# askerlee/segtran

Measured on NVIDIA H100. Metric: voxels/sec fwd+bwd Segtran3d BraTS 112^3 bs=4 hot path, higher is better.
Workload: dtype tf32

## Files before the change

segtran_b200/csrc/sx_gemm.cu:

```cuda
#include <algorithm>
#include <string>

#include "sx_common.cuh"
#include "sx_tc.cuh"

namespace {
using namespace sxtc;

constexpr int NUM_THREADS = 384;
constexpr int STAGES = 4;
constexpr int XPOSE_WARPS = 3;
constexpr int BN_WIDE = 256;
constexpr int CT_LD = 68;
constexpr int CT_WG_FLOATS = 32 * CT_LD;

template <int ES, bool A_MN, bool B_MN, int BN_T>
struct Plan {
  static_assert(BN_T == BN || (BN_T == BN_WIDE && ES == 4 && !A_MN && !B_MN),
                "sx_gemm: the 256-column tile is instantiated for K-major tf32 operands only");
  static constexpr int B_BYTES = BN_T * BKB;
  static constexpr int STAGE_BYTES = A_STAGE_BYTES + B_BYTES;
  static constexpr bool XA = ES == 4 && A_MN, XB = ES == 4 && B_MN;
  static constexpr bool XPOSE = XA || XB;
  static constexpr int RAW_BYTES = (XA ? A_STAGE_BYTES : 0) + (XB ? B_STAGE_BYTES : 0);
// ... 269 lines not shown
    for (int h = 0; h < 2; ++h) {
      const int grow = row0 + 8 * h + tr;
      const float* ar = base + zoff + (long long)(grow < p.M ? grow : 0) * p.ldc;
#pragma unroll
      for (int j = 0; j < 4; ++j) {
        const int col = col0 + 8 * j + tc;
        const int i0 = 4 * j + 2 * h;
        if (grow < p.M && col + 1 < p.N && p.c_vec_ok) {
          const float2 v = *reinterpret_cast<const float2*>(ar + col);
          g[i0] = v.x; g[i0 + 1] = v.y;
        } else {
          g[i0] = (grow < p.M && col < p.N) ? ar[col] : 0.f;
          g[i0 + 1] = (grow < p.M && col + 1 < p.N) ? ar[col + 1] : 0.f;
        }
      }
    }
  };

  const float drop_scale = p.drop_p > 0.f ? 1.f / (1.f - p.drop_p) : 1.f;
  const uint32_t drop_p16v = sx::drop_p16(p.drop_p);
  const unsigned long long drop_seed = p.drop_p > 0.f ? p.drop_seed + (p.drop_seed_dev ? *p.drop_seed_dev : 0ull) : 0ull;
  const uint32_t drop_mul_t = sx::drop_mul((tc >> 1) & 1), drop_key_t = sx::drop_key(drop_seed, (tc >> 1) & 1);

  float acc[BN_T / 2];
  for (int t = blockIdx.x; t < p.total_tiles; t += gridDim.x) {
    int z0, z1, mb, nb, ks;
    decode(t, z0, z1, mb, nb, ks);
    const int nq = p.z1_loop * split_kbs(ks);

    int prev = -1;
    for (int q = 0; q < nq; ++q) {
      sx::mbar_wait(&full_bar[stage], phase);
      const uint8_t* sa = smem + stage * STAGE_BYTES;
      const uint8_t* sb = sa + A_STAGE_BYTES;
      sx::acc_fence(acc);
      sx::wgmma_fence();
#pragma unroll
      for (int kk = 0; kk < KSTEPS; ++kk) {
        const uint64_t da = desc_a(sa, kk, A_MN && !kTF32), db = desc_b(sb, kk, B_MN && !kTF32);
        const uint32_t accum = (q > 0 || kk > 0) ? 1u : 0u;
        if constexpr (WIDE) sx::wgmma_tf32_n256(acc, da, db, accum);
        else if constexpr (kTF32) sx::wgmma_tf32(acc, da, db, accum);
        else sx::wgmma_bf16<A_MN ? 1 : 0, B_MN ? 1 : 0>(acc, da, db, accum);
      }
      sx::wgmma_commit();
      sx::acc_fence(acc);
      sx::wgmma_wait<1>();
      if (prev >= 0 && wtid == 0) sx::mbar_arrive(&empty_bar[prev]);
      prev = stage;
      if (++stage == STAGES) { stage = 0; phase ^= 1; }
    }
    sx::wgmma_wait<0>();
    sx::acc_fence(acc);
    if (prev >= 0 && wtid == 0) sx::mbar_arrive(&empty_bar[prev]);

    const long long zoff = (long long)z1 * p.c_sz1 + (long long)z0 * p.c_sz0;
    const float* bias = p.bias ? p.bias + (long long)z1 * p.bias_sz1 + (long long)z0 * p.bias_sz0 : nullptr;
    const bool add_bias = (bias != nullptr) && (ks == 0);
    const int row0 = mb * BM + cw * 64 + wq * 16;
    float tmax = -3.0e38f;
    float bias_m[2] = {0.f, 0.f};
    if (add_bias && p.bias_mode == SX_BIAS_M) {
#pragma unroll
      for (int h = 0; h < 2; ++h) {
        const int r = row0 + 8 * h + tr;
        bias_m[h] = r < p.M ? bias[r] : 0.f;
      }
    }
    constexpr int EPI_UNROLL = WIDE ? 1 : BN_T / 32;
#pragma unroll EPI_UNROLL
    for (int c = 0; c < BN_T / 32; ++c) {
      const int col0 = nb * BN_T + c * 32;
      if (col0 >= p.N) break;
      float f[16];
#pragma unroll
      for (int i = 0; i < 16; ++i) f[i] = acc[(WIDE ? 0 : 16 * c) + i] * p.alpha + bias_m[(i >> 1) & 1];
      if (p.addend) {
        float g[16];
        load_frag(p.addend, g, zoff, row0, col0);
#pragma unroll
        for (int i = 0; i < 16; ++i) f[i] += g[i];
      }
      if (add_bias && p.bias_mode == SX_BIAS_N) {
#pragma unroll
        for (int j = 0; j < 4; ++j) {
          const int col = col0 + 8 * j + tc;
          const float b0 = col < p.N ? bias[col] : 0.f, b1 = col + 1 < p.N ? bias[col + 1] : 0.f;
#pragma unroll
          for (int h = 0; h < 2; ++h) {
            f[4 * j + 2 * h] += b0;
            f[4 * j + 2 * h + 1] += b1;
          }
        }
      }
      auto apply_dropout = [&]() {
        if (p.drop_p > 0.f) {
          if (((p.ldc | zoff) & 3) == 0) {
#pragma unroll
            for (int h = 0; h < 2; ++h) {
              const unsigned long long g0 =
                  (unsigned long long)((zoff + (long long)(row0 + 8 * h + tr) * p.ldc + col0 + tc) >> 2);
#pragma unroll
              for (int j = 0; j < 4; ++j) {
                const uint32_t bits = sx::drop_word_k(drop_mul_t, drop_key_t, g0 + 2 * j);
                const int i0 = 4 * j + 2 * h;
                f[i0] = (bits & 0xFFFFu) >= drop_p16v ? f[i0] * drop_scale : 0.f;
                f[i0 + 1] = (bits >> 16) >= drop_p16v ? f[i0 + 1] * drop_scale : 0.f;
              }
            }
          } else {
#pragma unroll
            for (int h = 0; h < 2; ++h) {
              const long long rbase = zoff + (long long)(row0 + 8 * h + tr) * p.ldc;
#pragma unroll
              for (int j = 0; j < 4; ++j) {
                const unsigned long long e0 = (unsigned long long)(rbase + col0 + 8 * j + tc);
                const int i0 = 4 * j + 2 * h;
                f[i0] = sx::drop_keep1(drop_seed, e0, drop_p16v) ? f[i0] * drop_scale : 0.f;
                f[i0 + 1] = sx::drop_keep1(drop_seed, e0 + 1, drop_p16v) ? f[i0 + 1] * drop_scale : 0.f;
              }
            }
          }
        }
      };
      if (p.act == SX_ACT_GELU_BWD) {
        apply_dropout();
        float g[16];
        load_frag(reinterpret_cast<const float*>(p.preact), g, zoff, row0, col0);
#pragma unroll
        for (int i = 0; i < 16; ++i) f[i] *= sx::gelu_erf_grad(g[i]);
      } else {
        if (p.preact) store_frag(p.preact, f, zoff, row0, col0, false);
        if (p.act == SX_ACT_GELU) {
#pragma unroll
          for (int i = 0; i < 16; ++i) f[i] = sx::gelu_erf(f[i]);
        }
        apply_dropout();
      }
      if (p.round_tf32 && !p.c_bf16) {
#pragma unroll
        for (int i = 0; i < 16; ++i) f[i] = sx::round_tf32(f[i]);
      }
      if (p.amax) {
#pragma unroll
        for (int h = 0; h < 2; ++h)
          if (row0 + 8 * h + tr < p.M) {
#pragma unroll
            for (int j = 0; j < 4; ++j)
#pragma unroll
              for (int e = 0; e < 2; ++e)
                if (col0 + 8 * j + tc + e < p.N) tmax = fmaxf(tmax, f[4 * j + 2 * h + e]);
          }
      }
      if (!WIDE && p.split_k > 1) {
        float* pt = p.part + ((((long long)z1 * p.Z0 + z0) * p.tiles_m + mb) * p.tiles_n + nb) * p.split_k * (BM * BN) +
                    (long long)ks * (BM * BN);
#pragma unroll
        for (int h = 0; h < 2; ++h)
#pragma unroll
          for (int j = 0; j < 4; ++j)
            *reinterpret_cast<float2*>(pt + (row0 - mb * BM + 8 * h + tr) * BN + (col0 - nb * BN) + 8 * j + tc) =
                make_float2(f[4 * j + 2 * h], f[4 * j + 2 * h + 1]);
      } else {
        store_frag(p.C, f, zoff, row0, col0, p.accumulate != 0);
      }
      if constexpr (PL::CT) {
        if (p.ct) {
          float* cs = ct_stage + cw * CT_WG_FLOATS;
          named_bar_sync(1 + cw);
#pragma unroll
          for (int j = 0; j < 4; ++j)
#pragma unroll
            for (int h = 0; h < 2; ++h)
#pragma unroll
              for (int e = 0; e < 2; ++e) cs[(8 * j + tc + e) * CT_LD + wq * 16 + 8 * h + tr] = f[4 * j + 2 * h + e];
          named_bar_sync(1 + cw);
          const int m0 = mb * BM + cw * 64;
          const long long ctz = (long long)z1 * p.ct_sz1 + (long long)z0 * p.ct_sz0;
#pragma unroll
          for (int i = 0; i < 4; ++i) {
            const int v = wtid + 128 * i, n = v >> 4, r = (v & 15) * 4;
            const int gn = col0 + n, gm = m0 + r;
            if (gn < p.N && gm < p.M) {
              const float4 x = *reinterpret_cast<const float4*>(cs + n * CT_LD + r);
              float* o = p.ct + ctz + (long long)gn * p.ldct + gm;
              if (gm + 3 < p.M) {
                if (p.stream_out) __stcs(reinterpret_cast<float4*>(o), x);
                else *reinterpret_cast<float4*>(o) = x;
              } else {
                o[0] = x.x;
                if (gm + 1 < p.M) o[1] = x.y;
                if (gm + 2 < p.M) o[2] = x.z;
              }
            }
          }
        }
      }
      if constexpr (WIDE) {
#pragma unroll
        for (int i = 0; i < BN_T / 2 - 16; ++i) acc[i] = acc[i + 16];
      }
    }
    if (p.amax) {
      tmax = sx::warp_max(tmax);
      if (lane == 0 && tmax > -3.0e38f) sx::atomic_max_float(p.amax, tmax);
    }
  }
}

__global__ void split_reduce_kernel(const GemmParams p) {
  const long long total = (long long)p.total_tiles / p.split_k * (BM * BN);
  for (long long i = (long long)blockIdx.x * blockDim.x + threadIdx.x; i < total; i += (long long)gridDim.x * blockDim.x) {
    const int e = (int)(i % (BM * BN));
    long long t = i / (BM * BN);
    const int nb = (int)(t % p.tiles_n); t /= p.tiles_n;
    const int mb = (int)(t % p.tiles_m); t /= p.tiles_m;
    const int z0 = (int)(t % p.Z0), z1 = (int)(t / p.Z0);
    const int row = mb * BM + e / BN, col = nb * BN + e % BN;
    if (row >= p.M || col >= p.N) continue;
    const float* pt = p.part + (i / (BM * BN)) * p.split_k * (BM * BN) + e;
    float s = 0.f;
    for (int ks = 0; ks < p.split_k; ++ks) s += pt[(long long)ks * (BM * BN)];
    reinterpret_cast<float*>(p.C)[(long long)z1 * p.c_sz1 + (long long)z0 * p.c_sz0 + (long long)row * p.ldc + col] += s;
  }
}

long long g_max_ctas = -1;
int g_wide_tiles = -1;

template <int ES, bool A_MN, bool B_MN, int BN_T = BN>
int launch(const CUtensorMap& ta, const CUtensorMap& tb, const GemmParams& p, int grid, cudaStream_t st) {
  auto kern = sx_gemm_kernel<ES, A_MN, B_MN, BN_T>;
  constexpr int bytes = Plan<ES, A_MN, B_MN, BN_T>::SMEM;
  SX_CHECK_CUDA(set_max_smem_once(kern, bytes));
  kern<<<grid, NUM_THREADS, bytes, st>>>(ta, tb, p);
  SX_CHECK_CUDA(cudaGetLastError());
  if (p.split_k > 1) {
    const long long n = (long long)p.total_tiles / p.split_k * (BM * BN);
    split_reduce_kernel<<<(int)std::min<long long>(sx_ceil_div(n, 256), 65535), 256, 0, st>>>(p);
    SX_CHECK_CUDA(cudaGetLastError());
  }
  return 0;
}

}

extern "C" int sx_gemm_debug_set(const char* key, int64_t value) {
  std::string k(key);
  if (k == "max_ctas") g_max_ctas = value;
  else if (k == "wide_tiles") g_wide_tiles = value < 0 ? -1 : (value ? 1 : 0);
  else {
    sx_set_error("sx_gemm_debug_set: unknown key %s", key);
    return -1;
  }
  return 0;
}

static int gemm_run(const sx_gemm_args* a, const sx_gemm_tout* t, void* stream) {
  SX_REQUIRE(a != nullptr, "sx_gemm: null args");
  SX_REQUIRE(a->M > 0 && a->N > 0 && a->K > 0 && a->Z0 > 0 && a->Z1 > 0, "sx_gemm: bad shape M=%d N=%d K=%d Z=%dx%d",
             a->M, a->N, a->K, a->Z0, a->Z1);
  SX_REQUIRE(a->op_dtype == SX_OP_TF32 || a->op_dtype == SX_OP_BF16, "sx_gemm: bad op_dtype %d", a->op_dtype);
  SX_REQUIRE(a->C != nullptr && a->A.ptr != nullptr && a->B.ptr != nullptr, "sx_gemm: null pointer");
  const int es = a->op_dtype == SX_OP_TF32 ? 4 : 2;
  const int bk = BKB / es;
  const int sms = sm_count_cached();
  SX_REQUIRE(sms > 0, "sx_gemm: no CUDA device (this library has no CPU fallback)");

  GemmParams p{};
  p.M = a->M; p.N = a->N; p.K = a->K; p.Z0 = a->Z0; p.Z1 = a->Z1;
  p.tiles_m = sx_ceil_div(a->M, BM);
  p.tiles_n = sx_ceil_div(a->N, BN);
  p.num_kb = sx_ceil_div(a->K, bk);
  const bool fold_z1 = a->Z1 > 1 && a->c_stride_z1 == 0;
  SX_REQUIRE(!fold_z1 || (a->accumulate && !a->bias && !a->addend && a->act == SX_ACT_NONE && !a->preact && a->drop_p == 0.f),
             "sx_gemm: a z1-reduced output needs accumulate=1 and a linear epilogue without bias");
  p.z1_loop = fold_z1 ? a->Z1 : 1;
  p.Z1 = fold_z1 ? 1 : a->Z1;
  int split = a->split_k < 1 ? 1 : a->split_k;
  if (split > p.num_kb) split = p.num_kb;
  {
    const long long out_tiles = (long long)p.tiles_m * p.tiles_n * a->Z0 * p.Z1;
    const long long fit = a->part ? a->part_floats / ((long long)BM * BN * out_tiles) : 0;
    if (split > fit) split = fit < 2 ? 1 : (int)fit;
  }
  p.kb_per_split = sx_ceil_div(p.num_kb, split);
  p.split_k = sx_ceil_div(p.num_kb, p.kb_per_split);
  SX_REQUIRE(p.split_k == 1 || (a->accumulate && a->c_dtype == SX_F32 && a->act == SX_ACT_NONE && !a->preact &&
                                a->drop_p == 0.f && !a->amax),
             "sx_gemm: split_k > 1 needs accumulate=1 into fp32 C and a linear epilogue");
  SX_REQUIRE(!a->accumulate || a->c_dtype == SX_F32, "sx_gemm: accumulate needs fp32 C");
  SX_REQUIRE(!a->round_tf32 || (!a->accumulate && p.split_k == 1),
             "sx_gemm: round_tf32 cannot be combined with accumulate / split_k > 1 (a sum of rounded partials is not a TF32 "
             "value): round the finished output instead");
  const bool amn = a->A.major == SX_MAJOR_MN, bmn = a->B.major == SX_MAJOR_MN;
  const bool wide_legal = es == 4 && !amn && !bmn && p.split_k == 1;
  const long long wide_tt = (long long)p.tiles_m * sx_ceil_div(a->N, BN_WIDE) * a->Z0 * p.Z1;
  const bool wide = wide_legal && (g_wide_tiles == 1 || (g_wide_tiles < 0 && a->N > BN && 2 * wide_tt > sms));
  if (wide) p.tiles_n = sx_ceil_div(a->N, BN_WIDE);
  const long long tt = (long long)p.tiles_m * p.tiles_n * p.split_k * a->Z0 * p.Z1;
  SX_REQUIRE(tt < (1ll << 30), "sx_gemm: too many tiles");
  p.total_tiles = (int)tt;
  p.a_uses_z0 = a->A.stride_z0 != 0; p.a_uses_z1 = a->A.stride_z1 != 0;
  p.b_uses_z0 = a->B.stride_z0 != 0; p.b_uses_z1 = a->B.stride_z1 != 0;
  p.C = a->C; p.c_bf16 = a->c_dtype == SX_BF16; p.round_tf32 = a->round_tf32;
  p.ldc = a->ldc; p.c_sz0 = a->c_stride_z0; p.c_sz1 = a->c_stride_z1;
  p.c_vec_ok = ((reinterpret_cast<uintptr_t>(a->C) & 7) == 0) && (a->ldc % 2 == 0) && (a->c_stride_z0 % 2 == 0) &&
               (a->c_stride_z1 % 2 == 0) && (!a->preact || (reinterpret_cast<uintptr_t>(a->preact) & 7) == 0) &&
               (!a->addend || (reinterpret_cast<uintptr_t>(a->addend) & 7) == 0);
  p.alpha = a->alpha; p.bias_mode = a->bias ? a->bias_mode : SX_BIAS_NONE; p.bias = a->bias;
  p.bias_sz0 = a->bias_stride_z0; p.bias_sz1 = a->bias_stride_z1;
  p.act = a->act; p.accumulate = a->accumulate; p.preact = a->preact; p.amax = a->amax;
  p.addend = a->addend;
  SX_REQUIRE(a->act != SX_ACT_GELU_BWD || (a->preact && a->c_dtype == SX_F32 && p.split_k == 1 && !a->accumulate),
             "sx_gemm: SX_ACT_GELU_BWD needs the fp32 pre-activation in `preact`, fp32 C, split_k=1, accumulate=0");
  SX_REQUIRE(!a->addend || (p.split_k == 1 && !a->accumulate && a->c_dtype == SX_F32), "sx_gemm: addend needs split_k=1, accumulate=0, fp32 C");
  p.drop_p = a->drop_p; p.drop_seed = a->drop_seed;
  p.drop_seed_dev = reinterpret_cast<const unsigned long long*>(a->drop_seed_dev);
  if (t) {
    SX_REQUIRE(t->ct != nullptr, "sx_gemm: null ct");
    SX_REQUIRE(es == 4 && !amn && !bmn, "sx_gemm: ct needs tf32 operands, both K-major");
    SX_REQUIRE(p.split_k == 1 && !a->accumulate && a->c_dtype == SX_F32,
               "sx_gemm: ct needs split_k=1, accumulate=0, fp32 C");
    SX_REQUIRE((reinterpret_cast<uintptr_t>(t->ct) & 15) == 0 && t->ldct % 4 == 0 && t->ct_stride_z0 % 4 == 0 &&
                   t->ct_stride_z1 % 4 == 0 && t->ldct >= a->M,
               "sx_gemm: ct must be 16-byte aligned with ldct >= M and ldct, z strides multiples of 4");
    p.ct = t->ct; p.ldct = t->ldct; p.ct_sz0 = t->ct_stride_z0; p.ct_sz1 = t->ct_stride_z1;
  }
  {
    const double out_bytes =
        (double)a->M * a->N * a->Z0 * a->Z1 * (p.c_bf16 ? 2 : 4) * (1 + (a->preact ? 1 : 0) + (t ? 1 : 0));
    p.stream_out = out_bytes > 25.0 * 1024 * 1024;
  }

  CUtensorMap ta, tb;
  int rc = make_map(&ta, a->A, es, a->M, a->K, a->Z0, a->Z1, BM, "A");
  if (rc) return rc;
  rc = make_map(&tb, a->B, es, a->N, a->K, a->Z0, a->Z1, wide ? BN_WIDE : BN, "B");
  if (rc) return rc;

  int grid = p.total_tiles < sms ? p.total_tiles : sms;
  if (g_max_ctas > 0 && grid > g_max_ctas) grid = (int)g_max_ctas;
  p.part = a->part;
  cudaStream_t st = reinterpret_cast<cudaStream_t>(stream);
  if (wide) return launch<4, false, false, BN_WIDE>(ta, tb, p, grid, st);
  if (es == 4) {
    if (!amn && !bmn) return launch<4, false, false>(ta, tb, p, grid, st);
    if (!amn && bmn) return launch<4, false, true>(ta, tb, p, grid, st);
    if (amn && !bmn) return launch<4, true, false>(ta, tb, p, grid, st);
    return launch<4, true, true>(ta, tb, p, grid, st);
  }
  if (!amn && !bmn) return launch<2, false, false>(ta, tb, p, grid, st);
  if (!amn && bmn) return launch<2, false, true>(ta, tb, p, grid, st);
  if (amn && !bmn) return launch<2, true, false>(ta, tb, p, grid, st);
  return launch<2, true, true>(ta, tb, p, grid, st);
}

static thread_local sx_gemm_tout g_tout{};

extern "C" int sx_gemm_set_tout(const sx_gemm_tout* t) {
  g_tout = t ? *t : sx_gemm_tout{};
  SX_REQUIRE(t == nullptr || t->ct != nullptr, "sx_gemm_set_tout: null ct");
  return 0;
}

extern "C" int sx_gemm(const sx_gemm_args* a, void* stream) {
  const sx_gemm_tout t = g_tout;
  g_tout = sx_gemm_tout{};
  return gemm_run(a, t.ct ? &t : nullptr, stream);
}
```

segtran_b200/ops.py:

```python
from __future__ import annotations

import ctypes as C
import math
import os
from typing import Optional

import numpy as np
import torch

from . import _lib as L

_PRECISION = "tf32"


def set_precision(p: str):
    global _PRECISION
    if p not in ("tf32", "tf32x3", "bf16"):
        raise ValueError("unsupported precision %r (this build implements 'tf32', 'tf32x3' and 'bf16')" % (p,))
    _PRECISION = p
    _bf16_cache.clear()


def get_precision() -> str:
    return _PRECISION
# ... 294 lines not shown
        raise L.SxError("gemm_nt: bad output view %s %s" % (tuple(o4.shape), o4.stride()))
    g = L.sx_gemm_args()
    g.op_dtype = L.SX_OP_TF32
    if _PRECISION == "bf16":
        a4, b4 = _bf16_view(a4), _bf16_view(b4)
        g.op_dtype = L.SX_OP_BF16
    g.M, g.N, g.K, g.Z0, g.Z1 = M, N, K, Z0, Z1
    g.A = _operand(a4, Z1, Z0, "A")
    g.B = _operand(b4, Z1, Z0, "B")
    g.C = o4.data_ptr()
    g.c_dtype = L.SX_F32
    round_after = round_out and _PRECISION == "tf32" and (split_k > 1 or accumulate or reduce_z1)
    g.round_tf32 = 1 if (round_out and _PRECISION == "tf32" and not round_after) else 0
    g.ldc = o4.stride(-2)
    g.c_stride_z0 = o4.stride(1) if o4.shape[1] > 1 else 0
    g.c_stride_z1 = 0 if reduce_z1 else (o4.stride(0) if o4.shape[0] > 1 else 0)
    g.alpha = alpha
    if bias is not None:
        b4b = bias
        while b4b.dim() < 3:
            b4b = b4b.unsqueeze(0)
        g.bias = bias.data_ptr()
        g.bias_mode = bias_mode
        g.bias_stride_z0 = b4b.stride(1) if b4b.shape[1] > 1 else 0
        g.bias_stride_z1 = b4b.stride(0) if b4b.shape[0] > 1 else 0
    g.act = L.SX_ACT_GELU if gelu else L.SX_ACT_NONE
    if gelu_bwd is not None:
        if gelu or preact is not None or tuple(gelu_bwd.shape[-2:]) != (M, N) or gelu_bwd.stride() != out.stride():
            raise L.SxError("gemm_nt: gelu_bwd needs the pre-activation in the output's layout and no other activation")
        g.act = L.SX_ACT_GELU_BWD
        g.preact = gelu_bwd.data_ptr()
    g.split_k = split_k
    if split_k > 1:
        g.part, g.part_floats = _part_args(a.device)
    g.accumulate = 1 if (accumulate or reduce_z1 or split_k > 1) else 0
    if preact is not None:
        g.preact = preact.data_ptr()
    if amax is not None:
        g.amax = amax.data_ptr()
    g.drop_p = drop_p
    g.drop_seed, g.drop_seed_dev = _seed_args(seed)
    if addend is not None:
        if addend.dtype != torch.float32 or tuple(addend.shape[-2:]) != (M, N) or _as4(addend).stride() != o4.stride():
            raise L.SxError("gemm_nt: addend must be an fp32 tensor in the output's layout")
        g.addend = addend.data_ptr()
    if ct is not None:
        t4 = _as4(ct)
        if ct.dtype != torch.float32 or tuple(t4.shape[-2:]) != (N, M) or t4.stride(-1) != 1 or round_after:
            raise L.SxError("gemm_nt: ct must be an fp32 [..., N, M] view with m contiguous, on a single-pass product")
        t = L.sx_gemm_tout()
        t.ct = t4.data_ptr()
        t.ldct = t4.stride(-2)
        t.ct_stride_z0 = t4.stride(1) if t4.shape[1] > 1 else 0
        t.ct_stride_z1 = t4.stride(0) if t4.shape[0] > 1 else 0
        L.call("sx_gemm_set_tout", C.byref(t))
    L.call("sx_gemm", C.byref(g), _stream())
    if round_after and fresh:
        L.call("sx_convert", out.data_ptr(), L.SX_F32, out.numel(), out.data_ptr(), L.SX_F32, 1, _stream())
    return out


def gemm_nt(a: torch.Tensor, b: torch.Tensor, *, out: Optional[torch.Tensor] = None, alpha: float = 1.0,
            bias: Optional[torch.Tensor] = None, bias_mode: int = L.SX_BIAS_N, gelu: bool = False,
            preact: Optional[torch.Tensor] = None, accumulate: bool = False, split_k: Optional[int] = None,
            amax: Optional[torch.Tensor] = None, drop_p: float = 0.0, seed: int = 0, round_out: bool = True,
            reduce_z1: bool = False, gelu_bwd: Optional[torch.Tensor] = None,
            addend: Optional[torch.Tensor] = None, tag: str = "big", ct: Optional[torch.Tensor] = None) -> torch.Tensor:
    if not _three_pass(tag):
        return _gemm_nt_1(a, b, out=out, alpha=alpha, bias=bias, bias_mode=bias_mode, gelu=gelu, preact=preact,
                          accumulate=accumulate, split_k=split_k, amax=amax, drop_p=drop_p, seed=seed,
                          round_out=round_out, reduce_z1=reduce_z1, gelu_bwd=gelu_bwd, addend=addend, ct=ct)
    if ct is not None:
        raise L.SxError("gemm_nt: ct needs a single-pass product")
    _req_cuda(a, b)
    return _gemm_nt_1(_split_cat(a, 0), _split_cat(b, 1), out=out, alpha=alpha, bias=bias, bias_mode=bias_mode, gelu=gelu,
                      preact=preact, accumulate=accumulate, split_k=split_k, amax=amax, drop_p=drop_p, seed=seed,
                      round_out=round_out, reduce_z1=reduce_z1, gelu_bwd=gelu_bwd, addend=addend)


def _split_cat(t: torch.Tensor, role: int) -> torch.Tensor:
    t4 = _as4(t)
    Z1, Z0, R, K = t4.shape
    Kp = _pad4(K)
    out = torch.empty((Z1, Z0, R, 3 * Kp), device=t.device, dtype=torch.float32)
    L.call("sx_split_tf32_cat", t4.data_ptr(), Z1, Z0, R, K, t4.stride(0), t4.stride(1), t4.stride(2), t4.stride(3), Kp, role,
           out.data_ptr(), _stream())
    return out


def _pad4(n: int) -> int:
    return (n + 3) // 4 * 4


def _rowpad_empty(shape, device) -> torch.Tensor:
    Lr = shape[-1]
    buf = torch.empty(tuple(shape[:-1]) + (_pad4(Lr),), device=device, dtype=torch.float32)
    return buf[..., :Lr]


def _rows_ok(t: torch.Tensor) -> bool:
    if t.stride(-1) != 1 or t.stride(-2) % 4 != 0 or t.data_ptr() % 16 != 0:
        return False
    exp = t.stride(-2) * t.shape[-2]
    for d in range(t.dim() - 3, -1, -1):
        if t.shape[d] > 1 and t.stride(d) != exp:
            return False
        exp *= t.shape[d]
    return True


def _rowpad(t: torch.Tensor) -> torch.Tensor:
    if _rows_ok(t):
        return t
    o = _rowpad_empty(t.shape, t.device)
    o.copy_(t)
    return o


def round_tf32(x: torch.Tensor) -> torch.Tensor:
    _req_cuda(x)
    if _PRECISION == "tf32":
        r = getattr(x, "_sx_tf32", None)
        if r is not None and getattr(x, "_sx_tf32_version", -1) == x._version and \
                getattr(x, "_sx_tf32_ptr", None) == x.data_ptr():
            return r
    x = x.contiguous()
    if _PRECISION != "tf32":
        return x
    y = torch.empty_like(x)
    L.call("sx_convert", x.data_ptr(), L.SX_F32, x.numel(), y.data_ptr(), L.SX_F32, 1, _stream())
    return y


_KMAJOR_COPIES = os.environ.get("SEGTRAN_KMAJOR_COPIES", "1") != "0"


def set_kmajor_copies(on: bool):
    global _KMAJOR_COPIES
    _KMAJOR_COPIES = bool(on)


def _kmajor_copies(tag: str = "big") -> bool:
    return _KMAJOR_COPIES and _PRECISION == "tf32" and not _three_pass(tag)


def _transposed(x: torch.Tensor, Z: int, R: int, Cd: int) -> torch.Tensor:
    x = x.contiguous()
    y = _rowpad_empty((Z, Cd, R), x.device)
    L.call("sx_transpose", x.data_ptr(), Z, R, Cd, y.stride(1), y.data_ptr(), _stream())
    return y


def _token_kmajor(M: int, N: int, K: int, Z: int, tag: str = "big") -> bool:
    return _kmajor_copies(tag) and min(M, N) >= 512 and K >= 1024 and \
        2 * ((M + 127) // 128) * ((N + 255) // 256) * Z > 132


def _weight_t(Wr: torch.Tensor, Z: int, O: int, I: int) -> torch.Tensor:
    if _kmajor_copies():
        return _transposed(Wr, Z, O, I)
    return Wr.reshape(Z, O, I).transpose(-1, -2)


def colsum(x2d: torch.Tensor, out: Optional[torch.Tensor] = None) -> torch.Tensor:
    if out is None:
        out = _zeros((x2d.shape[1],), x2d.device)
    L.call("sx_colsum_batched", x2d.data_ptr(), 1, 0, 1, 0, x2d.shape[0], x2d.shape[1], x2d.stride(0), out.data_ptr(),
           *_part_args(x2d.device), _stream())
    return out


class _Linear(torch.autograd.Function):

    @staticmethod
    def forward(ctx, x, W, b, gelu, drop_p, seed, tag, round_y, addend):
        shp = x.shape
        x2 = x.reshape(-1, shp[-1])
        if not x2.is_contiguous():
            x2 = x2.contiguous()
        Wr = W.contiguous() if _three_pass(tag) else round_tf32(W)
        O = W.shape[0]
        y = torch.empty((x2.shape[0], O), device=x.device, dtype=torch.float32)
        h = torch.empty_like(y) if gelu else None
        a2 = None
        if addend is not None:
            a2 = addend.reshape(-1, O)
            if not a2.is_contiguous():
                a2 = a2.contiguous()
        gemm_nt(x2, Wr.view(O, -1), out=y, bias=b, gelu=gelu, preact=h, drop_p=drop_p, seed=seed, tag=tag,
                round_out=round_y, addend=a2)
        ctx.save_for_backward(x2, Wr, h)
        ctx.meta = (shp, b is not None, gelu, drop_p, seed, tag, None if addend is None else addend.shape)
        ctx.leaves = (W, b)
        return y.view(*shp[:-1], O)

    @staticmethod
    def backward(ctx, dy):
        x2, Wr, h = ctx.saved_tensors
        shp, has_b, gelu, drop_p, seed, tag, add_shape = ctx.meta
        W, b = ctx.leaves
        if _three_pass(tag) and _PRECISION == "tf32":
            Wr = round_tf32(W)
        O = W.shape[0]
        Wr2 = Wr.view(O, -1)
        dy2 = dy.reshape(-1, dy.shape[-1]).contiguous()
        if gelu or drop_p > 0:
            dh = torch.empty_like(dy2)
            L.call("sx_gelu_bwd", dy2.data_ptr(), _ptr(h), dy2.numel(), drop_p, *_seed_args(seed), dh.data_ptr(), _rt(),
                   _stream())
            dy2 = dh
        dx = dW = db = da = None
        if ctx.needs_input_grad[0]:
            dx = gemm_nt(dy2, _weight_t(Wr2, 1, *Wr2.shape)[0], round_out=False).view(shp)
        if ctx.needs_input_grad[1]:
            dW = _param_grad(W, dy2.t(), x2.t(), (O, -1))
        if has_b and ctx.needs_input_grad[2]:
            tgt = _grad_target(b)
            if tgt is not None:
                colsum(dy2, out=tgt)
            else:
                db = colsum(dy2)
        if add_shape is not None and ctx.needs_input_grad[8]:
            da = dy2.view(add_shape)
        return dx, dW, db, None, None, None, None, None, da


def linear(x, W, b=None, gelu=False, drop_p=0.0, seed=0, tag="big", round_out=True, addend=None):
    return _Linear.apply(x, W, b, gelu, drop_p, seed, tag, round_out, addend)


def _heads_aligned(dh: int, Fd: int) -> bool:
    es = 2 if _PRECISION == "bf16" else 4
    return (dh * es) % 16 == 0 and (Fd * es) % 16 == 0


def _head_rows(x: torch.Tensor, B: int, R: int, M: int, dh: int) -> torch.Tensor:
    v = x.view(B, R, M, dh).permute(0, 2, 1, 3)
    return v if _heads_aligned(dh, M * dh) else _rowpad(v)


def _head_cols(x: torch.Tensor, B: int, R: int, M: int, dh: int, kmajor: bool) -> torch.Tensor:
    if kmajor or not _heads_aligned(dh, M * dh):
        return _transposed(x, B, R, M * dh).unflatten(1, (M, dh))
    return x.view(B, R, M, dh).permute(0, 2, 3, 1)


class _AttnScores(torch.autograd.Function):

    @staticmethod
    def forward(ctx, q, k, M, amax, row_bias, tag, alpha=None):
        Bq, U1, Cq = q.shape
        B, U2 = k.shape[0], k.shape[1]
        d = Cq // M
        scale = 1.0 / math.sqrt(d) if alpha is None else float(alpha)
        qv = _head_rows(q, Bq, U1, M, d)
        kv = _head_rows(k, B, U2, M, d)
        S = _rowpad_empty((B, M, U1, U2), q.device)
        if row_bias is not None and M != 1:
            raise L.SxError("attn_scores: row_bias needs a single mode")
        rb = row_bias.contiguous().view(-1) if row_bias is not None else None
        gemm_nt(qv, kv, out=S, alpha=scale, amax=amax, round_out=False, bias=rb, bias_mode=L.SX_BIAS_M, tag=tag)
        ctx.save_for_backward(q, k)
        ctx.meta = (M, d, scale, row_bias.shape if row_bias is not None else None)
        ctx.tag = tag
        return S

    @staticmethod
    def backward(ctx, dS):
        q, k = ctx.saved_tensors
        M, d, scale, rb_shape = ctx.meta
        Bq, U1, Cq = q.shape
        B, U2 = k.shape[0], k.shape[1]
        dS = _rowpad(dS)
        dq, dk = _score_grads(dS, q, k, M, scale, ctx.needs_input_grad[0], ctx.needs_input_grad[1], ctx.tag)
        drb = None
        if rb_shape is not None and ctx.needs_input_grad[4]:
            drb = _zeros((U1,), q.device)
            L.call("sx_rowsum", dS.data_ptr(), B * U1, U2, dS.stride(-2), U1, drb.data_ptr(), *_part_args(dS.device), _stream())
            drb = drb.view(rb_shape)
        return dq, dk, None, None, drb, None, None


def _score_grads(dS, q, k, M, scale, need_q, need_k, tag="big", kmajor_k=False):
    Bq, U1, Cq = q.shape
    B, U2 = k.shape[0], k.shape[1]
    d = Cq // M
    dq = dk = None
    if need_q:
        bcast = Bq == 1 and B > 1
        dq = _zeros_like(q) if bcast else torch.empty_like(q)
        gemm_nt(dS, _head_cols(k, B, U2, M, d, kmajor_k), out=dq.view(Bq, U1, M, d).permute(0, 2, 1, 3), alpha=scale,
                round_out=False, reduce_z1=bcast, split_k=1, tag=tag)
    if need_k:
        dk = torch.empty_like(k)
        gemm_nt(dS.transpose(-1, -2), _head_cols(q, Bq, U1, M, d, False), out=dk.view(B, U2, M, d).permute(0, 2, 1, 3),
                alpha=scale, round_out=False, tag=tag)
    return dq, dk


class PosBias:
    __slots__ = ("table", "R", "grid", "w")

    def __init__(self, table, R, grid, w=1.0):
        grid = tuple(int(g) for g in grid)
        if len(grid) not in (2, 3) or table.dim() != len(grid) or any(s != 2 * R + 1 for s in table.shape):
            raise L.SxError("PosBias: table %s does not match radius %d over grid %s" % (tuple(table.shape), R, grid))
        self.table, self.R, self.grid, self.w = table, int(R), grid, float(w)

    def with_weight(self, w):
        return PosBias(self.table, self.R, self.grid, w)

    @property
    def num_tokens(self):
        n = 1
        for g in self.grid:
            n *= g
        return n


def _posbias_desc(table, R, grid, w) -> L.sx_posbias:
    d = L.sx_posbias()
    d.table = table.data_ptr()
    d.pd, d.R = len(grid), R
    for i, g in enumerate(grid):
        d.grid[i] = g
    d.w = w
    return d


def _posbias_table(pb):
    t = pb.table
    if t.dtype != torch.float32 or not t.is_contiguous():
        raise L.SxError("positional-bias table must be contiguous fp32")
    _req_cuda(t)
    return t


def attn_probs_fused(q, k, M, clip=500.0, drop_p=0.0, seed=0, diag=None, need_scores=False, round_out=True, posbias=None,
                     alpha=None):
    _req_cuda(q, k)
    if q.dtype != torch.float32 or k.dtype != torch.float32 or not q.is_contiguous() or not k.is_contiguous():
        raise L.SxError("attn_probs_fused: contiguous fp32 q/k expected")
    Bq, U1, Cq = q.shape
    B, U2, Ck = k.shape
    if Cq != Ck or Cq % M or (Cq // M) % 4 or Bq not in (1, B):
        raise L.SxError("attn_probs_fused: bad shapes q %s k %s modes %d" % (tuple(q.shape), tuple(k.shape), M))
    d = Cq // M
    P = _rowpad_empty((B, M, U1, U2), q.device)
    S = _rowpad_empty((B, M, U1, U2), q.device) if need_scores else None
    lse = torch.empty((B, M, U1), device=q.device, dtype=torch.float32)
    rowmax = torch.empty((B, M, U1), device=q.device, dtype=torch.float32)
    stat = _zeros((3,), q.device)
    a = L.sx_attn_probs_args()
    a.B, a.M, a.U1, a.U2, a.d = B, M, U1, U2, d
    a.round_tf32 = 1 if (round_out and _PRECISION == "tf32") else 0
    a.Q, a.q_ld, a.q_bstride = q.data_ptr(), Cq, (0 if Bq == 1 else U1 * Cq)
    a.K, a.k_ld, a.k_bstride = k.data_ptr(), Ck, U2 * Ck
    a.alpha, a.clip = (1.0 / math.sqrt(d) if alpha is None else float(alpha)), float(clip)
    a.P, a.S, a.ldp = P.data_ptr(), _ptr(S), P.stride(-2)
    a.lse, a.rowmax, a.stat, a.diag = lse.data_ptr(), rowmax.data_ptr(), stat.data_ptr(), _ptr(diag)
    a.drop_p = drop_p
    a.drop_seed, a.drop_seed_dev = _seed_args(seed)
    if posbias is not None:
        a.posbias = _posbias_desc(_posbias_table(posbias), posbias.R, posbias.grid, posbias.w)
    L.call("sx_attn_probs_fwd", C.byref(a), _stream())
    return P, S, lse, rowmax, stat


class _Scale(torch.autograd.Function):

    @staticmethod
    def forward(ctx, x, alpha):
        x = x.contiguous()
        y = torch.empty_like(x)
        L.call("sx_scale", x.data_ptr(), x.numel(), None, alpha, y.data_ptr(), _stream())
        ctx.alpha = alpha
        return y

    @staticmethod
    def backward(ctx, dy):
        return _Scale.apply(dy, ctx.alpha), None


def scale(x, alpha):
    return _Scale.apply(x, float(alpha))


class _Add(torch.autograd.Function):

    @staticmethod
    def forward(ctx, a, b):
        a, b = a.contiguous(), b.contiguous()
        y = torch.empty_like(a)
        L.call("sx_add", a.data_ptr(), b.data_ptr(), a.numel(), y.data_ptr(), _stream())
        return y

    @staticmethod
    def backward(ctx, dy):
        return dy, dy


def add(a, b):
    return _Add.apply(a, b)


class _MatVec(torch.autograd.Function):

    @staticmethod
    def forward(ctx, x, v):
        x = x.contiguous()
        v = v.contiguous()
        R, Cd = x.shape
        y = _sgemm(x, v, R, 1, Cd, (Cd, 1), (1, 1))[0].view(R)
        ctx.save_for_backward(x, v)
        return y

    @staticmethod
    def backward(ctx, dy):
        x, v = ctx.saved_tensors
        R, Cd = x.shape
        dy = dy.contiguous()
        dx = _sgemm(dy, v, R, Cd, 1, (1, 1), (1, 1))[0] if ctx.needs_input_grad[0] else None
        dv = _sgemm(dy, x, 1, Cd, R, (1, 1), (Cd, 1))[0].view(Cd) if ctx.needs_input_grad[1] else None
        return dx, dv


def matvec(x, v):
    return _MatVec.apply(x, v)


def softmax_posbias_backward(dP, ldd, S, lds, lse, R, Lr, amax, clip, drop_p, seed, ldp_fwd, dS, ldo, table, pb_geom,
                             table_needs_grad):
    tgt = _grad_target(table) if table_needs_grad else None
    buf = tgt if tgt is not None else _zeros((table.numel(),), table.device)
    L.call("sx_softmax_posbias_bwd", dP.data_ptr(), ldd, S.data_ptr(), lds, lse.data_ptr(), R, Lr, _ptr(amax), clip, drop_p,
           *_seed_args(seed), ldp_fwd, dS.data_ptr(), ldo, _rt(), C.byref(_posbias_desc(table, *pb_geom)), buf.data_ptr(),
           *_part_args(dS.device), _stream())
    if tgt is not None or not table_needs_grad:
        return None
    return buf.view(table.shape)


def softmax_backward(dP, S, lse, amax, clip, drop_p, seed, ldp, table=None, pb_geom=None, table_needs_grad=False):
    dP = _rowpad(dP)
    Lr = S.shape[-1]
    R = S.numel() // Lr
    dS = _rowpad_empty(S.shape, S.device)
    if table is None:
        L.call("sx_softmax_bwd", dP.data_ptr(), dP.stride(-2), S.data_ptr(), S.stride(-2), lse.data_ptr(), R, Lr,
               _ptr(amax), clip, drop_p, *_seed_args(seed), ldp, dS.data_ptr(), dS.stride(-2), _rt(), _stream())
        return dS, None
    return dS, softmax_posbias_backward(dP, dP.stride(-2), S, S.stride(-2), lse, R, Lr, amax, clip, drop_p, seed, ldp, dS,
                                        dS.stride(-2), table, pb_geom, table_needs_grad)


class _Softmax(torch.autograd.Function):

    @staticmethod
    def forward(ctx, S, amax, clip, drop_p, seed, diag, table, pb_geom):
        S = _rowpad(S)
        Lr, ld = S.shape[-1], S.stride(-2)
        R = S.numel() // Lr
        P = _rowpad_empty(S.shape, S.device)
        lse = torch.empty(R, device=S.device, dtype=torch.float32)
        args = (S.data_ptr(), R, Lr, ld, _ptr(amax), clip, drop_p, *_seed_args(seed), P.data_ptr(), P.stride(-2), _rt(),
                lse.data_ptr(), _ptr(diag))
        if table is None:
            L.call("sx_softmax_fwd", *args, _stream())
        else:
            L.call("sx_softmax_posbias_fwd", *args, C.byref(_posbias_desc(table, *pb_geom)), _stream())
        ctx.save_for_backward(S, lse, amax, table)
        ctx.meta = (clip, drop_p, seed, P.stride(-2), pb_geom)
        ctx.leaf = table
        return P

    @staticmethod
    def backward(ctx, dP):
        S, lse, amax, _table = ctx.saved_tensors
        clip, drop_p, seed, ldp, pb_geom = ctx.meta
        dS, dT = softmax_backward(dP, S, lse, amax, clip, drop_p, seed, ldp, ctx.leaf, pb_geom, ctx.needs_input_grad[6])
        return dS, None, None, None, None, None, dT, None


class _AttnPV(torch.autograd.Function):

    @staticmethod
    def forward(ctx, P, v, M, tag, round_out, heads):
        B, _, U1, U2 = P.shape
        Fd = v.shape[-1] // M
        P = _rowpad(P)
        if heads:
            U = torch.empty((B, U1, M * Fd), device=P.device, dtype=torch.float32)
            gemm_nt(P, _head_cols(v, B, U2, M, Fd, _kmajor_copies(tag)), out=U.view(B, U1, M, Fd).permute(0, 2, 1, 3),
                    tag=tag, round_out=round_out)
        else:
            vv = _head_cols(v, B, U2, M, Fd, _token_kmajor(U1, Fd, U2, B * M, tag))
            U = torch.empty((B, M, U1, Fd), device=P.device, dtype=torch.float32)
            gemm_nt(P, vv, out=U, tag=tag, round_out=round_out)
        ctx.save_for_backward(P, v)
        ctx.meta = (M, Fd, heads)
        ctx.tag = tag
        return U

    @staticmethod
    def backward(ctx, dU):
        P, v = ctx.saved_tensors
        M, Fd, heads = ctx.meta
        B, _, U1, U2 = P.shape
        dU = dU.contiguous()
        dP = dv = None
        if heads:
            if ctx.needs_input_grad[0]:
                dP = _rowpad_empty((B, M, U1, U2), P.device)
                gemm_nt(_head_rows(dU, B, U1, M, Fd), _head_rows(v, B, U2, M, Fd), out=dP, round_out=False, tag=ctx.tag)
            if ctx.needs_input_grad[1]:
                dv = torch.empty_like(v)
                gemm_nt(P.transpose(-1, -2), _head_cols(dU, B, U1, M, Fd, False),
                        out=dv.view(B, U2, M, Fd).permute(0, 2, 1, 3), round_out=False, tag=ctx.tag)
            return dP, dv, None, None, None, None
        dP, dv = _pv_grads(dU, P, v, M, Fd, ctx.needs_input_grad[0], ctx.needs_input_grad[1], ctx.tag)
        return dP, dv, None, None, None, None


def _pv_grads(dU, P, v, M, Fd, need_p, need_v, tag, dUt=None):
    B, _, U1, U2 = P.shape
    dP = dv = None
    if need_p:
        dP = _rowpad_empty((B, M, U1, U2), P.device)
        gemm_nt(dU, v.view(B, U2, M, Fd).permute(0, 2, 1, 3), out=dP, round_out=False, tag=tag)
    if need_v:
        dv = torch.empty_like(v)
        if dUt is None and _token_kmajor(U2, Fd, U1, B * M, tag):
            dUt = _transposed(dU, B * M, U1, Fd).unflatten(0, (B, M))
        if dUt is not None:
            Pt = _transposed(P, B * M, U1, U2).unflatten(0, (B, M))
            gemm_nt(Pt, dUt, out=dv.view(B, U2, M, Fd).permute(0, 2, 1, 3), round_out=False, tag=tag)
            del Pt
        else:
            gemm_nt(P.transpose(-1, -2), dU.transpose(-1, -2), out=dv.view(B, U2, M, Fd).permute(0, 2, 1, 3),
                    round_out=False, tag=tag)
    return dP, dv


class _FoldedValueBank(torch.autograd.Function):

    @staticmethod
    def forward(ctx, a, Wv, Wm, M, tag):
        B, A, Cd = a.shape
        Fd = Wm.shape[0]
        a2 = a.reshape(B * A, Cd)
        if not a2.is_contiguous():
            a2 = a2.contiguous()
        x3 = _three_pass(tag)
        Wvr = (Wv.contiguous() if x3 else round_tf32(Wv)).view(M, 1, Fd, Cd)
        Wmr = Wm.contiguous() if x3 else round_tf32(Wm)
        Wf = gemm_nt(Wmr.view(1, 1, Fd, Fd), Wvr.transpose(-1, -2), tag=tag, round_out=not x3)
        Vp = gemm_nt(a2, Wf.view(M * Fd, Cd), tag=tag)[0, 0]
        if x3 and _PRECISION == "tf32":
            Wf, Wvr, Wmr = round_tf32(Wf), round_tf32(Wv).view(M, 1, Fd, Cd), round_tf32(Wm)
        ctx.save_for_backward(a2, Wf, Wvr, Wmr)
        ctx.meta = (B, A, Cd, Fd, M)
        ctx.leaves = (Wv, Wm)
        return Vp.view(B, A, M * Fd)

    @staticmethod
    def backward(ctx, dVp):
        a2, Wf, Wvr, Wmr = ctx.saved_tensors
        B, A, Cd, Fd, M = ctx.meta
        Wv, Wm = ctx.leaves
        d2 = dVp.reshape(B * A, M * Fd)
        if not d2.is_contiguous():
            d2 = d2.contiguous()
        da = dWv = dWm = None
        if ctx.needs_input_grad[0]:
            da = gemm_nt(d2, _weight_t(Wf, 1, M * Fd, Cd)[0], round_out=False)[0, 0].view(B, A, Cd)
        if ctx.needs_input_grad[1] or ctx.needs_input_grad[2]:
            dWf = gemm_nt(d2.t(), a2.t(), round_out=False).view(M, 1, Fd, Cd)
            if ctx.needs_input_grad[2]:
                dWm = _param_grad(Wm, dWf, Wvr, (1, 1, Fd, Fd), reduce_z1=True)
            if ctx.needs_input_grad[1]:
                dWv = _param_grad(Wv, Wmr.t().view(1, 1, Fd, Fd), dWf.transpose(-1, -2), (M, 1, Fd, Cd))
        return da, dWv, dWm, None, None


def folded_value_bank(a, Wv, Wm, M, tag="small"):
    return _FoldedValueBank.apply(a, Wv, Wm, M, tag)


def _group_linear_fwd(G, Wo, bo):
    M, Fd = G.shape[1], G.shape[3]
    Wr = round_tf32(Wo).reshape(M, Fd, Fd)
    Y = torch.empty_like(G)
    gemm_nt(G, Wr.unsqueeze(0), out=Y, bias=bo.reshape(1, M, Fd), round_out=False)
    return Y, Wr


def _group_linear_param_grads(dY, G, Wo, bo, need_w, need_b, Gt=None):
    B, M, N, Fd = dY.shape
    dW = db = None
    if need_w:
        if Gt is not None:
            dYt = _transposed(dY, B * M, N, Fd).unflatten(0, (B, M))
            dW = _param_grad(Wo, dYt, Gt, (1, M, Fd, Fd), reduce_z1=True)
            del dYt
        else:
            dW = _param_grad(Wo, dY.transpose(-1, -2), G.transpose(-1, -2), (1, M, Fd, Fd), reduce_z1=True)
    if need_b:
        tgt = _grad_target(bo)
        buf = tgt if tgt is not None else _zeros((M * Fd,), dY.device)
        L.call("sx_colsum_batched", dY.data_ptr(), B, M * N * Fd, M, N * Fd, N, Fd, Fd, buf.data_ptr(),
               *_part_args(dY.device), _stream())
        db = None if tgt is not None else buf
    return dW, db


class _AttnPVGeluGroupLinear(torch.autograd.Function):

    @staticmethod
    def forward(ctx, P, v, M, bm, drop_p, seed, Wo, bo):
        B, _, U1, U2 = P.shape
        Fd = v.shape[-1] // M
        P = _rowpad(P)
        G = torch.empty((B, M, U1, Fd), device=P.device, dtype=torch.float32)
        H = torch.empty_like(G)
        kt = _token_kmajor(Fd, Fd, U1, M) and _token_kmajor(U2, Fd, U1, B * M)
        Gt = _rowpad_empty((B, M, Fd, U1), P.device) if kt else None
        gemm_nt(P, _head_cols(v, B, U2, M, Fd, _kmajor_copies()), out=G, bias=bm, gelu=True, preact=H, drop_p=drop_p,
                seed=seed, ct=Gt)
        Y, Wr = _group_linear_fwd(G, Wo, bo)
        ctx.save_for_backward(P, v, H, Gt if kt else G, Wr)
        ctx.meta = (M, Fd, drop_p, seed, kt)
        ctx.leaves = (bm, Wo, bo)
        return Y

    @staticmethod
    def backward(ctx, dY):
        P, v, H, G, Wr = ctx.saved_tensors
        M, Fd, drop_p, seed, kt = ctx.meta
        bm, Wo, bo = ctx.leaves
        dY = dY.contiguous()
        dbm_buf = dbm = None
        if bm is not None and ctx.needs_input_grad[3]:
            tgt = _grad_target(bm)
            dbm_buf = tgt if tgt is not None else _zeros((Fd,), dY.device)
            dbm = None if tgt is not None else dbm_buf
        dH = torch.empty_like(H)
        B, _, U1, _ = P.shape
        dHt = _rowpad_empty((B, M, Fd, U1), dY.device) if kt and ctx.needs_input_grad[1] else None
        gemm_nt(dY, _weight_t(Wr, M, Fd, Fd).unsqueeze(0), out=dH, gelu_bwd=H, drop_p=drop_p, seed=seed, ct=dHt)
        if dbm_buf is not None:
            colsum(dH.view(-1, Fd), out=dbm_buf)
        dW, dbo = _group_linear_param_grads(dY, None if kt else G, Wo, bo, ctx.needs_input_grad[6],
                                            ctx.needs_input_grad[7], Gt=G if kt else None)
        dP, dv = _pv_grads(dH, P, v, M, Fd, ctx.needs_input_grad[0], ctx.needs_input_grad[1], "big", dUt=dHt)
        return dP, dv, None, dbm, None, None, dW, dbo


def attn_pv_gelu_group_linear(P, v, M, bm, drop_p, seed, Wo, bo):
    return _AttnPVGeluGroupLinear.apply(P, v, M, bm, drop_p, seed, Wo, bo)


_ATTN_FUSION = True


def set_attn_fusion(on: bool):
    global _ATTN_FUSION
    _ATTN_FUSION = bool(on)


def attn_fusion_enabled() -> bool:
    return _ATTN_FUSION and _PRECISION == "tf32"


def _pb_args(posbias):
    if posbias is None:
        return None, None
    return _posbias_table(posbias), (posbias.R, posbias.grid, posbias.w)


class _LayerNorm(torch.autograd.Function):

    @staticmethod
    def forward(ctx, x, g, b, rnd, rnd_bwd):
        ctx.rnd_bwd = rnd_bwd
        x = x.contiguous()
        Cd = x.shape[-1]
        R = x.numel() // Cd
        y = torch.empty_like(x)
        stats = torch.empty((R, 2), device=x.device, dtype=torch.float32)
        L.call("sx_layernorm_fwd", x.data_ptr(), R, Cd, g.data_ptr(), b.data_ptr(), y.data_ptr(), rnd,
               stats.data_ptr(), _stream())
        ctx.save_for_backward(x, g, stats)
        ctx.leaves = (g, b)
        return y

    @staticmethod
    def backward(ctx, dy):
        x, g, stats = ctx.saved_tensors
        dy = dy.contiguous()
        Cd = x.shape[-1]
        R = x.numel() // Cd
        dx = torch.empty_like(x)
        dgb, dg = _sink_or_zeros(ctx.leaves[0])
        dbb, db = _sink_or_zeros(ctx.leaves[1])
        L.call("sx_layernorm_bwd", dy.data_ptr(), x.data_ptr(), R, Cd, g.data_ptr(), stats.data_ptr(), dx.data_ptr(),
               ctx.rnd_bwd, dgb.data_ptr(), dbb.data_ptr(), *_part_args(dy.device), _stream())
        return dx, dg, db, None, None


class _GroupLinear(torch.autograd.Function):

    @staticmethod
    def forward(ctx, G, Wo, bo):
        Y, Wr = _group_linear_fwd(G, Wo, bo)
        ctx.save_for_backward(G, Wr)
        ctx.leaves = (Wo, bo)
        return Y

    @staticmethod
    def backward(ctx, dY):
        G, Wr = ctx.saved_tensors
        B, M, N, Fd = G.shape
        dY = dY.contiguous()
        dG = None
        if ctx.needs_input_grad[0]:
            dG = gemm_nt(dY, _weight_t(Wr, M, Fd, Fd).unsqueeze(0), round_out=False)
        dW, db = _group_linear_param_grads(dY, G, *ctx.leaves, ctx.needs_input_grad[1], ctx.needs_input_grad[2])
        return dG, dW, db


class _LnSoftAggr(torch.autograd.Function):

    @staticmethod
    def forward(ctx, Y, g, b, ws, bs, drop_p, seed):
# ... 1113 lines not shown
```

Before: 533.7 million.

## Allow wide tiles with split-K and route more backward GEMMs through K-major copies

The 256-column wide tile path now supports split-K, with the partial buffer and reduce kernel templated on tile width. The fit and occupancy heuristics count split-K slices. On the Python side, several backward and weight-folding GEMMs (linear dW, attention dK, folded value bank dWf/dWv) now transpose operands into K-major copies when the heuristic allows, so they can use the tf32 wide-tile and ct epilogue path. This adds transpose copies and extra memory traffic in exchange for faster tensor-core GEMMs with non-transposing loads.

```diff
diff --git a/segtran_b200/csrc/sx_gemm.cu b/segtran_b200/csrc/sx_gemm.cu
--- a/segtran_b200/csrc/sx_gemm.cu
+++ b/segtran_b200/csrc/sx_gemm.cu
@@ -445,14 +445,14 @@
                 if (col0 + 8 * j + tc + e < p.N) tmax = fmaxf(tmax, f[4 * j + 2 * h + e]);
           }
       }
-      if (!WIDE && p.split_k > 1) {
-        float* pt = p.part + ((((long long)z1 * p.Z0 + z0) * p.tiles_m + mb) * p.tiles_n + nb) * p.split_k * (BM * BN) +
-                    (long long)ks * (BM * BN);
+      if (p.split_k > 1) {
+        float* pt = p.part + ((((long long)z1 * p.Z0 + z0) * p.tiles_m + mb) * p.tiles_n + nb) * p.split_k * (BM * BN_T) +
+                    (long long)ks * (BM * BN_T);
 #pragma unroll
         for (int h = 0; h < 2; ++h)
 #pragma unroll
           for (int j = 0; j < 4; ++j)
-            *reinterpret_cast<float2*>(pt + (row0 - mb * BM + 8 * h + tr) * BN + (col0 - nb * BN) + 8 * j + tc) =
+            *reinterpret_cast<float2*>(pt + (row0 - mb * BM + 8 * h + tr) * BN_T + (col0 - nb * BN_T) + 8 * j + tc) =
                 make_float2(f[4 * j + 2 * h], f[4 * j + 2 * h + 1]);
       } else {
         store_frag(p.C, f, zoff, row0, col0, p.accumulate != 0);
@@ -501,19 +501,21 @@
   }
 }
 
+template <int BN_T>
 __global__ void split_reduce_kernel(const GemmParams p) {
-  const long long total = (long long)p.total_tiles / p.split_k * (BM * BN);
+  constexpr int TILE = BM * BN_T;
+  const long long total = (long long)p.total_tiles / p.split_k * TILE;
   for (long long i = (long long)blockIdx.x * blockDim.x + threadIdx.x; i < total; i += (long long)gridDim.x * blockDim.x) {
-    const int e = (int)(i % (BM * BN));
-    long long t = i / (BM * BN);
+    const int e = (int)(i % TILE);
+    long long t = i / TILE;
     const int nb = (int)(t % p.tiles_n); t /= p.tiles_n;
     const int mb = (int)(t % p.tiles_m); t /= p.tiles_m;
     const int z0 = (int)(t % p.Z0), z1 = (int)(t / p.Z0);
-    const int row = mb * BM + e / BN, col = nb * BN + e % BN;
+    const int row = mb * BM + e / BN_T, col = nb * BN_T + e % BN_T;
     if (row >= p.M || col >= p.N) continue;
-    const float* pt = p.part + (i / (BM * BN)) * p.split_k * (BM * BN) + e;
+    const float* pt = p.part + (i / TILE) * p.split_k * TILE + e;
     float s = 0.f;
-    for (int ks = 0; ks < p.split_k; ++ks) s += pt[(long long)ks * (BM * BN)];
+    for (int ks = 0; ks < p.split_k; ++ks) s += pt[(long long)ks * TILE];
     reinterpret_cast<float*>(p.C)[(long long)z1 * p.c_sz1 + (long long)z0 * p.c_sz0 + (long long)row * p.ldc + col] += s;
   }
 }
@@ -529,8 +531,8 @@
   kern<<<grid, NUM_THREADS, bytes, st>>>(ta, tb, p);
   SX_CHECK_CUDA(cudaGetLastError());
   if (p.split_k > 1) {
-    const long long n = (long long)p.total_tiles / p.split_k * (BM * BN);
-    split_reduce_kernel<<<(int)std::min<long long>(sx_ceil_div(n, 256), 65535), 256, 0, st>>>(p);
+    const long long n = (long long)p.total_tiles / p.split_k * (BM * BN_T);
+    split_reduce_kernel<BN_T><<<(int)std::min<long long>(sx_ceil_div(n, 256), 65535), 256, 0, st>>>(p);
     SX_CHECK_CUDA(cudaGetLastError());
   }
   return 0;
@@ -573,8 +575,9 @@
   int split = a->split_k < 1 ? 1 : a->split_k;
   if (split > p.num_kb) split = p.num_kb;
   {
-    const long long out_tiles = (long long)p.tiles_m * p.tiles_n * a->Z0 * p.Z1;
-    const long long fit = a->part ? a->part_floats / ((long long)BM * BN * out_tiles) : 0;
+    const int fit_bn = es == 4 ? BN_WIDE : BN;
+    const long long out_tiles = (long long)p.tiles_m * sx_ceil_div(a->N, fit_bn) * a->Z0 * p.Z1;
+    const long long fit = a->part ? a->part_floats / ((long long)BM * fit_bn * out_tiles) : 0;
     if (split > fit) split = fit < 2 ? 1 : (int)fit;
   }
   p.kb_per_split = sx_ceil_div(p.num_kb, split);
@@ -587,8 +590,8 @@
              "sx_gemm: round_tf32 cannot be combined with accumulate / split_k > 1 (a sum of rounded partials is not a TF32 "
              "value): round the finished output instead");
   const bool amn = a->A.major == SX_MAJOR_MN, bmn = a->B.major == SX_MAJOR_MN;
-  const bool wide_legal = es == 4 && !amn && !bmn && p.split_k == 1;
-  const long long wide_tt = (long long)p.tiles_m * sx_ceil_div(a->N, BN_WIDE) * a->Z0 * p.Z1;
+  const bool wide_legal = es == 4 && !amn && !bmn;
+  const long long wide_tt = (long long)p.tiles_m * sx_ceil_div(a->N, BN_WIDE) * a->Z0 * p.Z1 * p.split_k;
   const bool wide = wide_legal && (g_wide_tiles == 1 || (g_wide_tiles < 0 && a->N > BN && 2 * wide_tt > sms));
   if (wide) p.tiles_n = sx_ceil_div(a->N, BN_WIDE);
   const long long tt = (long long)p.tiles_m * p.tiles_n * p.split_k * a->Z0 * p.Z1;
diff --git a/segtran_b200/ops.py b/segtran_b200/ops.py
--- a/segtran_b200/ops.py
+++ b/segtran_b200/ops.py
@@ -470,8 +470,9 @@
 
 
 def _token_kmajor(M: int, N: int, K: int, Z: int, tag: str = "big") -> bool:
-    return _kmajor_copies(tag) and min(M, N) >= 512 and K >= 1024 and \
-        2 * ((M + 127) // 128) * ((N + 255) // 256) * Z > 132
+    if not (_kmajor_copies(tag) and min(M, N) >= 512 and K >= 1024):
+        return False
+    return 2 * ((M + 127) // 128) * ((N + 255) // 256) * Z * _pick_split_k(M, N, K, Z) > 132
 
 
 def _weight_t(Wr: torch.Tensor, Z: int, O: int, I: int) -> torch.Tensor:
@@ -531,7 +532,11 @@
         if ctx.needs_input_grad[0]:
             dx = gemm_nt(dy2, _weight_t(Wr2, 1, *Wr2.shape)[0], round_out=False).view(shp)
         if ctx.needs_input_grad[1]:
-            dW = _param_grad(W, dy2.t(), x2.t(), (O, -1))
+            T, I = x2.shape
+            if _token_kmajor(O, I, T, 1):
+                dW = _param_grad(W, _transposed(dy2, 1, T, O)[0], _transposed(x2, 1, T, I)[0], (O, -1))
+            else:
+                dW = _param_grad(W, dy2.t(), x2.t(), (O, -1))
         if has_b and ctx.needs_input_grad[2]:
             tgt = _grad_target(b)
             if tgt is not None:
@@ -611,8 +616,14 @@
                 round_out=False, reduce_z1=bcast, split_k=1, tag=tag)
     if need_k:
         dk = torch.empty_like(k)
-        gemm_nt(dS.transpose(-1, -2), _head_cols(q, Bq, U1, M, d, False), out=dk.view(B, U2, M, d).permute(0, 2, 1, 3),
-                alpha=scale, round_out=False, tag=tag)
+        if _token_kmajor(U2, d, U1, B * M, tag):
+            dSt = _transposed(dS, B * M, U1, U2).unflatten(0, (B, M))
+            gemm_nt(dSt, _head_cols(q, Bq, U1, M, d, True), out=dk.view(B, U2, M, d).permute(0, 2, 1, 3), alpha=scale,
+                    round_out=False, tag=tag)
+            del dSt
+        else:
+            gemm_nt(dS.transpose(-1, -2), _head_cols(q, Bq, U1, M, d, False),
+                    out=dk.view(B, U2, M, d).permute(0, 2, 1, 3), alpha=scale, round_out=False, tag=tag)
     return dq, dk
 
 
@@ -872,7 +883,10 @@
         x3 = _three_pass(tag)
         Wvr = (Wv.contiguous() if x3 else round_tf32(Wv)).view(M, 1, Fd, Cd)
         Wmr = Wm.contiguous() if x3 else round_tf32(Wm)
-        Wf = gemm_nt(Wmr.view(1, 1, Fd, Fd), Wvr.transpose(-1, -2), tag=tag, round_out=not x3)
+        if _token_kmajor(Fd, Cd, Fd, M, tag):
+            Wf = gemm_nt(Wmr.view(1, 1, Fd, Fd), _transposed(Wvr, M, Fd, Cd).unsqueeze(1), tag=tag, round_out=not x3)
+        else:
+            Wf = gemm_nt(Wmr.view(1, 1, Fd, Fd), Wvr.transpose(-1, -2), tag=tag, round_out=not x3)
         Vp = gemm_nt(a2, Wf.view(M * Fd, Cd), tag=tag)[0, 0]
         if x3 and _PRECISION == "tf32":
             Wf, Wvr, Wmr = round_tf32(Wf), round_tf32(Wv).view(M, 1, Fd, Cd), round_tf32(Wm)
@@ -893,11 +907,23 @@
         if ctx.needs_input_grad[0]:
             da = gemm_nt(d2, _weight_t(Wf, 1, M * Fd, Cd)[0], round_out=False)[0, 0].view(B, A, Cd)
         if ctx.needs_input_grad[1] or ctx.needs_input_grad[2]:
-            dWf = gemm_nt(d2.t(), a2.t(), round_out=False).view(M, 1, Fd, Cd)
+            kf = _token_kmajor(M * Fd, Cd, B * A, 1) and _pick_split_k(M * Fd, Cd, B * A, 1) == 1
+            kv = kf and ctx.needs_input_grad[1] and _token_kmajor(Fd, Cd, Fd, M) and Fd % 4 == 0
+            dWft = _rowpad_empty((Cd, M * Fd), d2.device) if kv else None
+            if kf:
+                dWf = gemm_nt(_transposed(d2, 1, B * A, M * Fd)[0], _transposed(a2, 1, B * A, Cd)[0], round_out=False,
+                              ct=dWft)
+            else:
+                dWf = gemm_nt(d2.t(), a2.t(), round_out=False)
+            dWf = dWf.view(M, 1, Fd, Cd)
             if ctx.needs_input_grad[2]:
                 dWm = _param_grad(Wm, dWf, Wvr, (1, 1, Fd, Fd), reduce_z1=True)
             if ctx.needs_input_grad[1]:
-                dWv = _param_grad(Wv, Wmr.t().view(1, 1, Fd, Fd), dWf.transpose(-1, -2), (M, 1, Fd, Cd))
+                if kv:
+                    dWv = _param_grad(Wv, _transposed(Wmr, 1, Fd, Fd).unsqueeze(1),
+                                      dWft.unflatten(1, (M, Fd)).permute(1, 0, 2).unsqueeze(1), (M, 1, Fd, Cd))
+                else:
+                    dWv = _param_grad(Wv, Wmr.t().view(1, 1, Fd, Fd), dWf.transpose(-1, -2), (M, 1, Fd, Cd))
         return da, dWv, dWm, None, None
 
 
```

New measurement: 546.1 million, median of 6. 2.3% higher.
